# DataZooDE/anofox-forecast

Measured on AMD Instinct MI355X. Metric: series/sec fit+forecast, AutoETS h=28 on M5-shape batches, higher is better.
Workload: dtype f64

## Files before the change

anofox-forecast_amd/csrc/ets_fit_kernel.hpp:

```cpp
#pragma once
#include "ets_device.hpp"
#include "classic_device.hpp"
#include "kernels.hpp"

#ifndef ANOFOX_ROUND_WAVES
#define ANOFOX_ROUND_WAVES 2
#endif
namespace anofox {

#ifndef ANOFOX_PARK_CLASS
#define ANOFOX_PARK_CLASS 0
#endif
#ifndef ANOFOX_PARK_WAVES
#define ANOFOX_PARK_WAVES 4
#endif
#ifndef ANOFOX_DM_WPB
#define ANOFOX_DM_WPB 1
#endif
#ifndef ANOFOX_SETPRIO
#define ANOFOX_SETPRIO 0
#endif
#ifndef ANOFOX_ROUND_WAVES_COMPACT
#define ANOFOX_ROUND_WAVES_COMPACT ANOFOX_ROUND_WAVES
#endif
#ifndef ANOFOX_SEQ_WAVES_COMPACT
#define ANOFOX_SEQ_WAVES_COMPACT 0
#endif
template <class Cfg, class YT = double> struct RoundTraits {
    static constexpr bool DAMPED_MUL = !Cfg::CLASSIC && Cfg::T == C_MUL && Cfg::D;
    static constexpr bool PARK = !Cfg::CLASSIC && (ANOFOX_PARK_CLASS >= 3 || (ANOFOX_PARK_CLASS == 2 && !Cfg::ADDITIVE) || (ANOFOX_PARK_CLASS == 1 && DAMPED_MUL));
    static constexpr int WAVES = PARK ? ANOFOX_PARK_WAVES : (std::is_same_v<YT, double> ? ANOFOX_ROUND_WAVES : ANOFOX_ROUND_WAVES_COMPACT);
    static constexpr int WPB = DAMPED_MUL ? ANOFOX_DM_WPB : 1;
};

template <class Cfg, int MS, class YT = double, bool CLASSIC = Cfg::CLASSIC> struct RoundModelOf { using type = EtsModel<Cfg, MS, 1, YT>; };
template <class Cfg, int MS, class YT> struct RoundModelOf<Cfg, MS, YT, true> { using type = ClassicRoundModel<Cfg::KIND, MS>; };

template <class Cfg, int MS, int SPEC, bool K4 = false, class YT = double>
__device__ __forceinline__ void ets_round_body(const FitArgs &a, const int vblock, const int vgrid, const int wave, double *const lds_all)
{
    constexpr int D = Cfg::DIM;
    constexpr bool PARK = RoundTraits<Cfg>::PARK;
    if constexpr (ANOFOX_SETPRIO >= 1 && RoundTraits<Cfg>::DAMPED_MUL) __builtin_amdgcn_s_setprio(3);
    else if constexpr (ANOFOX_SETPRIO >= 2 && !Cfg::CLASSIC && !Cfg::ADDITIVE) __builtin_amdgcn_s_setprio(ANOFOX_SETPRIO == 2 ? 1 : 2);
    if (a.wave_prio == 3) __builtin_amdgcn_s_setprio(3);
    else if (a.wave_prio == 2) __builtin_amdgcn_s_setprio(2);
    else if (a.wave_prio == 1) __builtin_amdgcn_s_setprio(1);
    if constexpr (Cfg::T == C_MUL && Cfg::D) dm_pow_tab_init();
    const int lane = threadIdx.x & (NM_BLOCK - 1);
    const int lds_per_wave = (PARK ? 0 : nm_lds_doubles<D>()) + ((MS == -1 || MS == -3) ? a.m * NM_BLOCK : 0);
    double *const lds = lds_all + (size_t)wave * (size_t)lds_per_wave;
    double *const nmst = PARK ? a.nm_scratch + (size_t)vblock * (size_t)nm_lds_doubles<D>() : lds;
    double *const lds_ring = PARK ? lds : lds + nm_lds_doubles<D>();
    const unsigned long long trace_t0 = a.wave_trace ? __builtin_amdgcn_s_memrealtime() : 0ull;
    const int n_act = a.n_active ? *a.n_active : a.n_series;
    int mode = SPEC;
    if constexpr (SPEC == 3) mode = n_act > a.spec_below ? 0 : ((a.spec2_below > 0 && n_act <= a.spec2_below && n_act <= vgrid) ? 2 : 1);
    else if (a.spec_below >= 0) {
        const int owner = n_act > a.spec_below ? 0 : (n_act > a.spec2_below ? 1 : 2);
        if (owner != SPEC) return;
    }
    const int LPP = mode == 0 ? 1 : (mode == 1 ? NM_K : NM_BLOCK);
    const int PPB = NM_BLOCK / LPP;
    if (vblock * PPB >= n_act) return;
    const int p = vblock * PPB + lane / LPP;
    const bool valid = p < n_act;
    const int s = valid ? (a.series_of ? a.series_of[p] : p) : 0;
    const int len = valid ? a.len[s] : 0;

    const int m = a.m_col ? (MS <= -3 ? a.m_col[s] : __builtin_amdgcn_readfirstlane(a.m_col[s])) : a.m;
    const int n_param = a.n_param - ((Cfg::S != C_NONE && a.m_col) ? a.m - m : 0);
    bool active = valid;
    if (!a.first_round && a.series_of == nullptr && valid && a.st.done[s]) active = false;
    if (a.first_round) {
        int st = FIT_OK;
        if constexpr (Cfg::CLASSIC) {
            const int min_len = Cfg::KIND == CK_HW ? 2 * m : (Cfg::KIND == CK_SEASONAL_ES ? m : a.min_len);
            if (len <= 0 || (a.mask != nullptr && valid && a.mask[s] != a.want)) st = FIT_SKIPPED;
            else if (len < min_len) st = FIT_SHORT;
        } else {
            const uint32_t fl = valid ? a.flags[s] : 0u;
            if (len <= 0) st = FIT_SKIPPED;
            else if (Cfg::S != C_NONE && len < 2 * m) st = FIT_SHORT;
            else if (len < n_param + 2) st = FIT_SHORT;
            else if (a.need_positive && !(fl & SF_POSITIVE)) st = FIT_NONPOSITIVE;
            else if (a.skip_constant && (fl & SF_CONSTANT)) st = FIT_SKIPPED;
        }
        active = valid && st == FIT_OK;
        if (valid) {
            a.status[s] = st;
            if (!active) { a.st.done[s] = 1; a.st.passes[s] = 0; a.st.evals[s] = 0; a.st.iters[s] = 0; }
        }
    }

    SeriesView v;
// ... 14 lines not shown
    mdl.in.b0 = (active && !Cfg::CLASSIC && Cfg::T != C_NONE) ? a.b0[s] : 0.0;
    mdl.in.fig = a.fig ? a.fig + s : nullptr;
    mdl.in.fig_ld = a.fig_ld;
    mdl.in.m = m;
    mdl.ring = (MS == -2 || MS == -4) ? a.ring_scratch + (size_t)vblock * (size_t)a.m * NM_BLOCK : lds_ring;

    NmRun r;
    if (a.first_round) nm_init_simplex(mdl, nmst, r, active);
    else {
#pragma unroll
        for (int k = 0; k <= D; k++) {
#pragma unroll
            for (int i = 0; i < D; i++) nmst[(k * D + i) * NM_BLOCK + lane] = active ? a.st.sim[(size_t)(k * D + i) * a.ld + s] : 0.0;
            nmst[((D + 1) * D + k) * NM_BLOCK + lane] = active ? a.st.fs[(size_t)k * a.ld + s] : 0.0;
        }
        r.phase = active ? a.st.phase[s] : NM_ITER;
        r.evals = active ? a.st.evals[s] : 0;
        r.iters = active ? a.st.iters[s] : 0;
        r.passes = active ? a.st.passes[s] : 0;
        r.done = !active;
    }
    const int passes_in = r.passes;

    const int budget = mode == 2 ? (1 << 30) : ((SPEC == 3 && mode == 0 && !K4) ? a.budget_seq : a.budget);
#define ANOFOX_ADVANCE_LANE()                                                                          \
    do {                                                                                               \
        if constexpr (K4) {                                                                            \
            EtsModel<Cfg, MS, NM_K, YT> mdl4;                                                          \
            mdl4.v = mdl.v; mdl4.in = mdl.in; mdl4.ring = mdl.ring;                                    \
            nm_advance_spec(mdl4, nmst, r, budget);                                                    \
        } else nm_advance_seq(mdl, nmst, r, budget);                                                   \
    } while (0)
    if constexpr (SPEC == 3) {
        if (mode == 2) nm_advance_spec2(mdl, nmst, r, budget);
        else if (mode == 1) nm_advance_spec(mdl, nmst, r, budget);
        else ANOFOX_ADVANCE_LANE();
    } else if constexpr (SPEC == 2) nm_advance_spec2(mdl, nmst, r, budget);
    else if constexpr (SPEC == 1) nm_advance_spec(mdl, nmst, r, budget);
    else ANOFOX_ADVANCE_LANE();
#undef ANOFOX_ADVANCE_LANE
    nm_fence();

    if (a.wave_trace && lane == 0) {
        const unsigned long long slot = atomicAdd(a.wave_trace, 1ull);
        if (slot < a.wave_trace[1]) {
            unsigned long long *rec = a.wave_trace + 4 + 4 * slot;
            rec[0] = a.wave_trace_tag | ((unsigned long long)mode << 8) | (unsigned long long)(K4 ? 4 : 0);
            rec[1] = trace_t0;
            rec[2] = __builtin_amdgcn_s_memrealtime();
            rec[3] = (unsigned long long)__builtin_amdgcn_s_getreg(0xF804) | ((unsigned long long)__builtin_amdgcn_s_getreg(0xF814) << 32);
        }
    }
    if (a.lane_stats) {
        const int mine = r.passes - passes_in;
        int sum = mine;
#pragma unroll
        for (int o = 32; o >= 1; o >>= 1) sum += __shfl_xor(sum, o);
        const int most = wave_max_i32(mine);
        if (lane == 0 && most > 0) {
            atomicAdd(a.lane_stats, (unsigned long long)most);
            atomicAdd(a.lane_stats + 1, (unsigned long long)sum);
        }
    }
    if (active && (lane % LPP) == 0) {
#pragma unroll
        for (int k = 0; k <= D; k++) {
#pragma unroll
// ... 91 lines not shown
        }
        return;
    }

    if (want_sd && valid && len > 0) a.sd_out[s] = active ? sqrt(var / (double)len) : 0.0;
    if (valid && len > 0) {
        double aicc = __builtin_huge_val();
        if (active) {
            const double lik = f[0];
            if (!(fabs(lik) <= 1.7976931348623157e308)) { st = FIT_NONFINITE; a.status[s] = st; }
            else {
                const double dk = (double)n_param, dn = (double)len;
                const double aic = lik + 2.0 * dk;
                aicc = aic + 2.0 * dk * (dk + 1.0) / (dn - dk - 1.0);
            }
        }
        a.aicc[s] = aicc;
        a.evals[s] = active ? a.st.evals[s] : 0;
        a.iters[s] = active ? a.st.iters[s] : 0;
        a.passes[s] = active ? a.st.passes[s] + 1 : 0;
    }
}

template <class Cfg, int MS, int SPEC, bool K4 = false, class YT = double>
void ets_round_launch(const FitArgs &a, hipStream_t stream)
{
    static_assert(!K4 || ((SPEC == 0 || SPEC == 3) && MS >= 0 && !Cfg::CLASSIC), "K4: the one-lane-per-problem driver of an ETS spec without a run-time ring");
    constexpr int PPB = SPEC == 0 ? NM_BLOCK : (SPEC == 1 ? NM_BLOCK / NM_K : 1);
    int grid;
    if (SPEC == 3) {
        const int n = a.n_series;
        const int g_seq = (n + NM_BLOCK - 1) / NM_BLOCK;
        const int g_spec = (std::min(n, std::max(a.spec_below, 0)) + NM_BLOCK / NM_K - 1) / (NM_BLOCK / NM_K);
        const int g_spec2 = std::min(n, std::max(a.spec2_below, 0));
        grid = std::max(g_seq, std::max(g_spec, g_spec2));
    } else {
        const int n_max = (SPEC == 2 && a.spec_below >= 0 && a.spec2_below < a.n_series) ? a.spec2_below : a.n_series;
        grid = (n_max + PPB - 1) / PPB;
    }
    if (grid <= 0) return;
    constexpr int WPB = RoundTraits<Cfg>::WPB;
    const int blocks = (grid + WPB - 1) / WPB;
    if (RoundTraits<Cfg>::PARK && (a.nm_scratch == nullptr || (size_t)blocks * WPB * (size_t)nm_lds_doubles<Cfg::DIM>() > a.nm_scratch_doubles))
        throw std::runtime_error("ets_round_launch: the simplex scratch does not cover the launch");
    if ((MS == -2 || MS == -4) && (a.ring_scratch == nullptr || (size_t)blocks * WPB * (size_t)a.m * NM_BLOCK > a.ring_scratch_doubles))
        throw std::runtime_error("ets_round_launch: the seasonal-ring scratch does not cover the launch");
    size_t lds_bytes = RoundTraits<Cfg>::PARK ? 0 : sizeof(double) * (size_t)nm_lds_doubles<Cfg::DIM>();
    if (MS == -1 || MS == -3) lds_bytes += sizeof(double) * (size_t)a.m * NM_BLOCK;
    lds_bytes *= WPB;
    if (lds_bytes > 48 * 1024)
        anofox_check_attr(hipFuncSetAttribute((const void *)ets_round_kernel<Cfg, MS, SPEC, K4, YT>, hipFuncAttributeMaxDynamicSharedMemorySize, (int)lds_bytes));
    hipLaunchKernelGGL((ets_round_kernel<Cfg, MS, SPEC, K4, YT>), dim3(blocks), dim3(NM_BLOCK * WPB), lds_bytes, stream, a);
}

template <class Cfg, int MS, class YT = double>
void ets_final_launch(const FitArgs &a, hipStream_t stream)
{
    const int grid = (a.n_series + NM_BLOCK - 1) / NM_BLOCK;
    if (MS == -2 && (a.ring_scratch == nullptr || (size_t)grid * (size_t)a.m * NM_BLOCK > a.ring_scratch_doubles))
        throw std::runtime_error("ets_final_launch: the seasonal-ring scratch does not cover the launch");
    size_t lds_bytes = (MS == -1) ? sizeof(double) * (size_t)a.m * NM_BLOCK : 0;
    hipLaunchKernelGGL((ets_final_kernel<Cfg, MS, YT>), dim3(grid), dim3(NM_BLOCK), lds_bytes, stream, a);
}

}
```

anofox-forecast_amd/csrc/host_api.hip:

```cpp
#include <hip/hip_runtime.h>

#include <algorithm>
#include <cctype>
#include <atomic>
#include <memory>
#include <unordered_map>
#include <chrono>
#include <cmath>
#include <condition_variable>
#include <mutex>
#include <cstdio>
#include <cstdlib>
#include <cstring>
#include <limits>
#include <map>
#include <stdexcept>
#include <string>
#include <system_error>
#include <thread>
#include <vector>

#include "classic_device.hpp"
#include "host_semantics.hpp"
#include "kernels.hpp"
// ... 539 lines not shown
    a.yhat = b->d_yhat; a.status = b->d_detail; a.passes = b->d_passes_total;
    a.model_code = code; a.model_code_out = write_code ? b->d_model_code : nullptr;
    a.ring_scratch = nullptr;
    a.m_col = (kind == CK_HW || kind == CK_SEASONAL_ES) ? b->d_m_col : nullptr;
    const bool optimise = kind == CK_HOLT || kind == CK_HW || optimized != 0;
    if (optimise) {
        const size_t n = b->n, ld = b->ld;
        if (!b->classic_st.sim) {
            b->classic_st.sim = dalloc<double>(12 * ld); b->classic_st.fs = dalloc<double>(4 * ld);
            b->classic_st.phase = dalloc<int32_t>(ld); b->classic_st.evals = dalloc<int32_t>(ld); b->classic_st.iters = dalloc<int32_t>(ld);
            b->classic_st.passes = dalloc<int32_t>(ld); b->classic_st.done = dalloc<int32_t>(ld);
            b->d_classic_status = dalloc<int32_t>(ld);
            b->classic_map[0] = dalloc<int32_t>(ld); b->classic_map[1] = dalloc<int32_t>(ld); b->classic_cnt = dalloc<int32_t>(3);
        }
        double *ybuf = (b->n_slots_cap > 0 && b->use_gather) ? b->lanes[0].ybuf : nullptr;
        size_t ybuf_cols = ybuf ? b->lanes[0].ybuf_cols : ld;
        if (!ybuf) {
            const double per_col = (double)std::max<size_t>(b->t_max, 1) * 8.0;
            const size_t cols = (size_t)std::min((double)ld, 32.0 * 1073741824.0 / per_col) / 64 * 64;
            if (cols >= 1024 || cols >= ld) {
                if (!b->d_classic_ybuf) { b->d_classic_ybuf = dalloc<double>(std::max<size_t>(b->t_max, 1) * cols); b->classic_ybuf_cols = cols; }
                ybuf = b->d_classic_ybuf;
                ybuf_cols = b->classic_ybuf_cols;
            }
        }
        const bool seasonal = kind == CK_HW || kind == CK_SEASONAL_ES;
        FitArgs f{};
        f.y = b->d_y; f.ld = ld; f.len = d_len; f.n_series = (int)n; f.t_rows = (int)std::max<size_t>(b->t_max, 1);
        f.m = seasonal ? std::max(m, 1) : 1; f.h = b->h;
        f.flags = b->d_flags; f.fig = nullptr; f.fig_ld = ld;
        f.status = b->d_classic_status; f.st = b->classic_st;
        f.mask = mask; f.want = want; f.min_len = min_len;
        f.m_col = a.m_col;
        const bool merged = f.m_col != nullptr;
        FitLaunchers fns = classic_fit_launcher(kind, (merged && f.m == 7) ? 8 : f.m);
        if (!fns.round_seq || !fns.round_spec || !fns.round_spec2 || !fns.round_auto) throw HipFail{"no round kernel for this model"};
        if (f.m > ETS_LDS_PERIOD) {
            const size_t wg = merged ? n : std::max<size_t>((n + 15) / 16, std::min<size_t>(n, 1024));
            f.ring_scratch = ensure_ring(b, wg * (size_t)f.m * 64u);
            f.ring_scratch_doubles = wg * (size_t)f.m * 64u;
        }
        static const int BUDGET[] = {24, 24, 24, 24, 48, 48, 96, 192, 1024};
        const bool tiny = n <= TINY_BATCH_PROBLEMS;
        const int n_rounds = tiny ? 1 : (merged ? (n > 4096 ? 4 : 3) : (int)(sizeof BUDGET / sizeof BUDGET[0]));
        for (int r = 0; r < n_rounds; r++) {
            f.first_round = (r == 0);
            f.spec_below = -1; f.spec2_below = -1;
            f.gathered = 0;
            f.y_round = b->d_y; f.ld_round = ld; f.series_of = nullptr; f.n_active = nullptr;
            if (tiny) {
                f.budget = 1 << 30; f.budget_seq = f.budget;
                fns.round_spec2(f, st);
            } else if (merged) {
                f.budget = r == 0 ? 64 : (r == 1 ? 128 : 256); f.budget_seq = f.budget;
                (r < n_rounds - 1 ? fns.round_spec : fns.round_spec2)(f, st);
            } else if (r == 0) {
                const bool seq0 = n >= 4u * 65536u;
                f.budget = seq0 ? (BUDGET[0] * 7) / 4 : BUDGET[0];
                (seq0 ? fns.round_seq : fns.round_spec)(f, st);
            } else {
                int32_t **map = b->classic_map, *cnt = b->classic_cnt;
                const int32_t *prev_map = (r == 1) ? nullptr : map[(r - 1) & 1];
                const int32_t *prev_cnt = (r == 1) ? nullptr : cnt + ((r - 1) % 3);
                if (r == 1) HIPCHECK(hipMemsetAsync(cnt, 0, 3 * sizeof(int32_t), st));
                launch_compact(prev_map, prev_cnt, (int)n, b->classic_st.done, map[r & 1], cnt + (r % 3), st, cnt + ((r + 1) % 3));
                f.series_of = map[r & 1]; f.n_active = cnt + (r % 3);
// ... 196 lines not shown
    std::stable_sort(order.begin(), order.end(), [&](size_t x, size_t y) { return work(specs[x]) > work(specs[y]); });
    std::vector<int> stream_of(order.size());
    for (size_t oi = 0; oi < order.size(); oi++) stream_of[oi] = (int)(oi % (size_t)n_lanes);
    std::vector<FitArgs> args(order.size());
    std::vector<FitLaunchers> fns(order.size());
    for (size_t oi = 0; oi < order.size(); oi++) {
        const size_t k = order[oi];
        const int id = specs[k];
        const int q = (int)(oi % (size_t)n_lanes);
        auto &lane = b->lanes[q];
        const int se = spec_season(id), ti = spec_trend_idx(id);
        const int tt = ti == 0 ? 0 : (ti <= 2 ? 1 : 2);
        FitArgs &a = args[oi];
        a = FitArgs{};
        a.y = (const double *)ybase; a.ld = ld; a.len = d_len; a.n_series = (int)n; a.t_rows = (int)std::max<size_t>(b->t_max, 1);
        a.m = se != 0 ? m : 1; a.h = b->h;
        a.l0 = b->d_l0 + (size_t)(se * 3 + tt) * ld;
        a.b0 = b->d_b0 + (size_t)(se * 3 + tt) * ld;
        a.fig = se == 1 ? b->d_fig_add : (se == 2 ? b->d_fig_mul : nullptr);
        a.fig_ld = ld;
        a.flags = b->d_flags;
        a.need_positive = spec_has_mult(id) ? 1 : 0;
        a.skip_constant = skip_constant ? 1 : 0;
        a.n_param = spec_n_param(id, a.m);
        a.aicc = b->d_aicc + k * ld;
        a.yhat = b->d_yhat_slots + k * n * (size_t)b->h;
        a.status = b->d_status_slots + k * ld;
        a.evals = b->d_evals_slots + k * ld;
        a.iters = b->d_iters_slots + k * ld;
        a.passes = b->d_passes_slots + k * ld;
        a.st = lane.st;
        a.ring_scratch = nullptr;
        a.m_col = b->d_m_col;
        if (b->sd_in_final && order.size() == 1) { a.mean = b->d_mean; a.sd_out = b->d_sd; }
        a.lane_stats = b->d_lane_stats ? b->d_lane_stats + 2 * k : nullptr;
        a.wave_trace = b->d_wave_trace;
        fns[oi] = ets_fit_launcher(id, (merged && se != 0) ? (a.m > lds_limit ? ETS_PERLANE_HBM : ETS_PERLANE_LDS) : a.m, yt);
        if (!fns[oi].round_seq || !fns[oi].round_spec || !fns[oi].round_auto || !fns[oi].final) throw HipFail{"no kernel for ETS spec id " + std::to_string(id)};
    }
    {
        size_t n_long = 0;
        for (size_t oi = 0; oi < order.size(); oi++) if (args[oi].m > lds_limit) n_long++;
        if (n_long) {
            const bool tiny_batch = (uint64_t)n * order.size() <= (uint64_t)TINY_BATCH_PROBLEMS;
            const size_t wg = std::max<size_t>((n + 15) / 16, std::min<size_t>(n, tiny_batch ? n : (size_t)std::max(b->spec2_below, b->spec2_below_md)));
            const size_t per_spec = wg * (size_t)m * 64u;
            if ((double)n_long * (double)per_spec * 8.0 > 64.0 * 1073741824.0)
                throw HipFail{"seasonal period " + std::to_string(m) + " on " + std::to_string(n) + " series needs more than 64 GiB of ring scratch: shard the batch"};
            double *base = ensure_ring(b, n_long * per_spec);
            size_t k = 0;
            for (size_t oi = 0; oi < order.size(); oi++) if (args[oi].m > lds_limit) { args[oi].ring_scratch = base + (k++) * per_spec; args[oi].ring_scratch_doubles = per_spec; }
        }
    }
    {
        const bool tiny_batch = (uint64_t)n * order.size() <= (uint64_t)TINY_BATCH_PROBLEMS;
        const size_t wg = std::max<size_t>((n + 15) / 16, std::min<size_t>(n, tiny_batch ? n : (size_t)std::max(b->spec2_below, b->spec2_below_md)));
        for (size_t oi = 0; oi < order.size(); oi++) {
            if (!fns[oi].nm_scratch_per_wg) continue;
            auto &lane = b->lanes[oi % (size_t)n_lanes];
            const size_t need = (wg + 8) * fns[oi].nm_scratch_per_wg;
            if (lane.nm_scratch_doubles < need) {
                if (lane.nm_scratch) b->retired.push_back(lane.nm_scratch);
                lane.nm_scratch = nullptr; lane.nm_scratch_doubles = 0;
                lane.nm_scratch = dalloc<double>(need);
                lane.nm_scratch_doubles = need;
            }
            args[oi].nm_scratch = lane.nm_scratch; args[oi].nm_scratch_doubles = lane.nm_scratch_doubles;
        }
    }
    std::vector<char> dead(order.size(), 0);
    if (b->none_pos && !b->fixed_params)
        for (size_t oi = 0; oi < order.size(); oi++)
            if (args[oi].need_positive) dead[oi] = 1;
    std::vector<char> k4(order.size(), 0);
    {
        bool all_additive = true;
        for (size_t oi = 0; oi < order.size(); oi++)
            if (!dead[oi] && spec_has_mult(specs[order[oi]]) && !(b->live_all > 0 && b->live_pos >= 0 && 2 * (int64_t)b->live_pos < (int64_t)b->live_all))
                all_additive = false;
        int64_t additive_live = 0;
        for (size_t oi = 0; oi < order.size(); oi++)
            if (!dead[oi] && !spec_has_mult(specs[order[oi]])) additive_live += b->live_all >= 0 ? (int64_t)b->live_all : (int64_t)n;
        int64_t all_live = 0;
        for (size_t oi = 0; oi < order.size(); oi++)
            if (!dead[oi]) all_live += (spec_has_mult(specs[order[oi]]) && b->live_pos >= 0) ? (int64_t)b->live_pos : (b->live_all >= 0 ? (int64_t)b->live_all : (int64_t)n);
        const bool on = b->tun.k4 > 0 || (b->tun.k4 < 0 && yt == YT_F64 && ((all_additive && additive_live >= 131072) || all_live >= 524288));
        for (size_t oi = 0; oi < order.size(); oi++)
            k4[oi] = on && !dead[oi] && !b->fixed_params && !spec_has_mult(specs[order[oi]]) && fns[oi].round_k4 && fns[oi].round_auto_k4;
    }
// ... 92 lines not shown
            if (b->tun.group_split == 2) add_split(of_class[GROUP_GENERAL], GROUP_GENERAL);
            else add(of_class[GROUP_GENERAL], GROUP_GENERAL);
            add(of_class[GROUP_ADDITIVE], GROUP_ADDITIVE);
            grouped = !groups.empty();
        }
        if (grouped) {
            for (size_t g = 0; g < groups.size(); g++) {
                const bool dm = spec_trend_idx(specs[order[groups[g][0]]]) == 4;
                group_stream.push_back(dm ? (int)g : N_AUX_STREAMS - 1 - (int)g);
                for (size_t oi : groups[g]) { group_of[oi] = (int)g; stream_of[oi] = group_stream[g]; slot_of[oi] = n_slots++; }
            }
            for (size_t oi = 0; oi < order.size(); oi++) if (dead[oi]) stream_of[oi] = group_stream[0];
        }
    }
    bool emit = true;
    std::vector<int> slot_blocks, slot_k4;
    GroupCompactArgs gc{};
    GroupGatherArgs gg{};
    int gg_cols = 0;
    auto run_round = [&](const size_t oi, const int kind, const FitArgs &a, hipStream_t sq, const int r) {
        if (!grouped) {
            const FitLaunchFn f = kind == RK_SEQ ? fns[oi].round_seq : kind == RK_SPEC ? fns[oi].round_spec : kind == RK_SPEC2 ? fns[oi].round_spec2 :
                                  kind == RK_AUTO ? fns[oi].round_auto : kind == RK_K4 ? fns[oi].round_k4 : fns[oi].round_auto_k4;
            f(a, sq);
            return;
        }
        if (emit) return;
        FitArgs t = a;
        if (kind == RK_SEQ || kind == RK_K4) { t.spec_below = -1; t.spec2_below = -1; t.budget_seq = t.budget; }
        else if (kind == RK_SPEC) { t.spec_below = 0x7fffffff; t.spec2_below = -1; }
        else if (kind == RK_SPEC2) throw HipFail{"launch_fit_slots: the one-wave-per-problem round of a tiny batch has no group form"};
        const int g_seq = (int)((n + NM_BLOCK - 1) / NM_BLOCK);
        const int g_spec = (int)((std::min<int64_t>((int64_t)n, std::max(t.spec_below, 0)) + NM_BLOCK / NM_K - 1) / (NM_BLOCK / NM_K));
        const int g_spec2 = (int)std::min<int64_t>((int64_t)n, std::max(t.spec2_below, 0));
        const int blocks = std::max(g_seq, std::max(g_spec, g_spec2));
        if (t.ring_scratch != nullptr && (size_t)blocks * (size_t)t.m * NM_BLOCK > t.ring_scratch_doubles)
            throw HipFail{"launch_fit_slots: the seasonal-ring scratch does not cover a group slot"};
        const size_t cell = (size_t)r * n_slots + slot_of[oi];
        b->h_group_tab[cell] = t;
        slot_blocks[cell] = blocks;
        slot_k4[cell] = (kind == RK_K4 || kind == RK_AUTO_K4) ? 1 : 0;
    };
    auto enqueue_round = [&](const int r, const size_t oi) {
            if (dead[oi]) return;
            const int q = (int)(oi % (size_t)n_lanes);
            auto &lane = b->lanes[q];
            hipStream_t sq = spec_stream(stream_of[oi]);
            FitArgs &a = args[oi];
            const bool spec_mode = r >= b->seq_rounds;
            a.first_round = (r == 0);
            a.wave_trace_tag = ((unsigned long long)specs[order[oi]] << 32) | ((unsigned long long)r << 16);
            a.wave_prio = (int)oi < b->tun.prio_top ? std::max(1, 3 - (int)oi) : 0;
            a.spec_below = -1; a.spec2_below = -1;
            a.gathered = 0;
            if (tiny) {
                a.y_round = b->d_y; a.ld_round = ld; a.series_of = nullptr; a.n_active = nullptr;
                a.budget = 1 << 30; a.budget_seq = a.budget;
                run_round(oi, RK_SPEC2, a, sq, r);
                b->fit_launches++;
                return;
            }
            if (r == 0 && b->use_pos && a.need_positive) {
                if (emit)
                    hipLaunchKernelGGL(retire_nonpositive_kernel, dim3((unsigned)((n + 255) / 256)), dim3(256), 0, sq, (int)n, d_len, b->d_notpos,
                                       a.status, lane.st.done, lane.st.passes, lane.st.evals, lane.st.iters);
                a.series_of = b->d_pos_map; a.n_active = b->d_pos_cnt;
                if (b->d_ypos) { a.y_round = b->d_ypos; a.ld_round = ld; a.gathered = 1; a.gather_cap = (int)ld; }
// ... 4513 lines not shown
```

anofox-forecast_amd/csrc/host_resources.hpp:

```cpp
#pragma once

constexpr int N_AUX_STREAMS = 32;

struct HipFail { std::string msg; bool oom = false; };
void report_hip_failure(AnofoxError *out_error, const HipFail &f)
{
    if (f.oom) anofox::set_error(out_error, ALLOCATION_ERROR, "Allocation error: " + f.msg);
    else anofox::set_error(out_error, INTERNAL_ERROR, "Internal error: " + f.msg);
}
#define HIPCHECK(expr)                                                                             \
    do {                                                                                           \
        hipError_t _e = (expr);                                                                    \
        if (_e != hipSuccess) throw HipFail{std::string(#expr) + ": " + hipGetErrorString(_e), _e == hipErrorOutOfMemory};    \
    } while (0)

#define LAUNCHCHECK(what)                                                                          \
    do {                                                                                           \
        hipError_t _e = hipGetLastError();                                                         \
        if (_e != hipSuccess) throw HipFail{std::string("kernel launch failed (") + (what) + "): " + hipGetErrorString(_e), false};    \
    } while (0)

constexpr int32_t STATUS_NOT_COMPUTED = -1;

struct Tunables {
    std::vector<int> budgets{24, 24, 24, 24, 24, 24, 48, 48, 96, 96, 192, 1024};
    int seq_rounds = -1;
    int gather_cols = 0;
    int gather = -1;
    int spec_below = 8192;
    int spec_below_md = 8192;
    int spec2_below = 1024;
    int spec2_below_md = 2048;
    int k4 = -1;
    int k4_top = 1, k4_top_below = 20480;
    std::string wave_trace;
    int compact = -1;
    int fill_policy = 1;
    int fill_target = 150;
    int fill_late_div = 2;
    int fill_s2_div = 16;
    int top_boost_n = 0, top_boost_pct = 200;
    int prio_top = 0;
    int group_launch = 1;
    int group_split = 1;
    int dm_head_rounds = 0;
    bool merge_periods = true;
    int part_threads = 16;
    int pack_threads = 0;
    bool timing = false;
    int arima_trace = 0;
    double arima_lookahead = 6.0;
    int arima_lookahead_depth = 2;
    double arima_spec_factor = 4.0;
    double arima_shared_chunk_rounds = 1.0;
    int arima_prep_lanes = 64;
    int arima_queue_sort = 1;
    int arima_refit_budget = 100;
    static std::map<std::string, std::string> tune_map()
    {
        std::map<std::string, std::string> kv;
        const char *e = std::getenv("ANOFOX_HIP_TUNE");
        if (!e) return kv;
        std::string all(e);
        for (size_t pos = 0; pos < all.size();) {
            size_t end = all.find(';', pos);
// ... 9 lines not shown
            pos = end + 1;
        }
        return kv;
    }
    static Tunables from_env()
    {
        Tunables t;
        const std::map<std::string, std::string> kv = tune_map();
        auto geti = [&](const char *k, int &v) { auto it = kv.find(k); if (it != kv.end()) v = std::atoi(it->second.c_str()); };
        auto getd = [&](const char *k, double &v) { auto it = kv.find(k); if (it != kv.end()) v = std::atof(it->second.c_str()); };
        if (kv.count("budgets")) {
            std::vector<int> v;
            for (const char *q = kv.at("budgets").c_str(); *q;) {
                char *end = nullptr;
                long x = std::strtol(q, &end, 10);
                if (end == q) break;
                if (x > 0) v.push_back((int)x);
                q = (*end == ',') ? end + 1 : end;
            }
            if (!v.empty()) t.budgets = v;
        }
        if (kv.count("wave_trace")) t.wave_trace = kv.at("wave_trace");
        geti("compact", t.compact); geti("prio_top", t.prio_top); geti("top_boost_n", t.top_boost_n); geti("top_boost_pct", t.top_boost_pct);
        geti("fill_policy", t.fill_policy); geti("fill_target", t.fill_target); geti("fill_late_div", t.fill_late_div); geti("fill_s2_div", t.fill_s2_div);
        geti("seq_rounds", t.seq_rounds);
        geti("gather", t.gather);
        if (kv.count("spec_below")) t.spec_below = t.spec_below_md = std::atoi(kv.at("spec_below").c_str());
        geti("spec_below_md", t.spec_below_md);
        geti("gather_cols", t.gather_cols);
        geti("group_launch", t.group_launch); geti("group_split", t.group_split);
        geti("k4", t.k4); geti("dm_head_rounds", t.dm_head_rounds); geti("k4_top", t.k4_top); geti("k4_top_below", t.k4_top_below);
        if (kv.count("spec2_below")) t.spec2_below = t.spec2_below_md = std::atoi(kv.at("spec2_below").c_str());
        geti("spec2_below_md", t.spec2_below_md);
        if (kv.count("merge_periods")) t.merge_periods = std::atoi(kv.at("merge_periods").c_str()) != 0;
        geti("part_threads", t.part_threads);
        if (kv.count("arima_trace")) t.arima_trace = std::atoi(kv.at("arima_trace").c_str());
        getd("arima_lookahead", t.arima_lookahead);
        geti("arima_lookahead_depth", t.arima_lookahead_depth);
        getd("arima_spec_factor", t.arima_spec_factor);
        geti("arima_queue_sort", t.arima_queue_sort);
        geti("arima_prep_lanes", t.arima_prep_lanes);
        getd("arima_shared_chunk_rounds", t.arima_shared_chunk_rounds);
        geti("arima_refit_budget", t.arima_refit_budget);
        if (const char *e = std::getenv("ANOFOX_HIP_PACK_THREADS")) t.pack_threads = std::max(1, std::atoi(e));
        t.timing = std::getenv("ANOFOX_HIP_TIMING") != nullptr;
        return t;
    }
};
struct ProcessTunables {
    double cache_gb = -1.0, pinned_cache_gb = 2.0;
    double coalesce_us = 1000.0;
    int prio_streams = -1;
    std::string devices;
    static const ProcessTunables &get()
    {
        static const ProcessTunables t = [] {
            ProcessTunables p;
            if (const char *e = std::getenv("ANOFOX_HIP_CACHE_GB")) p.cache_gb = std::atof(e);
            if (const char *e = std::getenv("ANOFOX_HIP_PINNED_CACHE_GB")) p.pinned_cache_gb = std::atof(e);
            { const auto kv = Tunables::tune_map(); auto it = kv.find("prio_streams"); if (it != kv.end()) p.prio_streams = std::atoi(it->second.c_str()); }
            if (const char *e = std::getenv("ANOFOX_HIP_COALESCE_US")) p.coalesce_us = std::atof(e);
            if (const char *e = std::getenv("ANOFOX_HIP_DEVICES")) p.devices = e;
            return p;
        }();
        return t;
    }
// ... 423 lines not shown
```

anofox-forecast_amd/csrc/kernels.hpp:

```cpp
#pragma once
#include <hip/hip_runtime.h>
#include <stddef.h>
#include <stdint.h>
#include <atomic>

#include <stdexcept>
#include <string>

namespace anofox {

inline void anofox_check_attr(hipError_t e)
{
    if (e != hipSuccess) throw std::runtime_error(std::string("launch preparation failed: ") + hipGetErrorString(e));
}

enum : uint32_t { SF_POSITIVE = 1u, SF_CONSTANT = 2u, SF_HAS_NAN = 4u };

enum : int32_t { FIT_OK = 0, FIT_SHORT = 1, FIT_NONPOSITIVE = 2, FIT_NONFINITE = 3, FIT_PERIOD = 4, FIT_SKIPPED = 5 };

struct PrepArgs {
    const double *y; size_t ld; const int32_t *len; int n_series;
    int m;
    const int32_t *m_col;
    double *mean, *sd;
    uint32_t *flags;
    double *fig_add, *fig_mul;
    double *l0, *b0;
    double *scratch;
    int pre_fig;
    int t_rows;
    int skip_sd;
    int skip_types;
};

size_t season_scratch_doubles(int n_series, int t_rows, int m_max);
void launch_season_figures(const PrepArgs &a, hipStream_t stream);

struct NmStateBuf {
    double *sim;
    double *fs;
    int32_t *phase, *evals, *iters, *passes, *done;
};

struct FitArgs {
    const double *y; size_t ld; const int32_t *len; int n_series;
    int t_rows;
    const double *y_round; size_t ld_round;
    const int32_t *series_of;
    const int32_t *n_active;
    int budget, first_round;
    const int32_t *m_col;
    int spec_below;
    const uint32_t *mask;
    uint32_t want;
    int min_len;
    int budget_seq;
    int spec2_below;
    int gathered;
    int gather_cap;
    NmStateBuf st;
    double *ring_scratch;
    size_t ring_scratch_doubles;
    double *nm_scratch;
    size_t nm_scratch_doubles;
    int m, h;
    const double *l0, *b0;
    const double *fig; size_t fig_ld;
    const uint32_t *flags;
    int need_positive;
    int skip_constant;
    int n_param;
    double *aicc;
    double *yhat;
    int32_t *status;
    int32_t *evals, *iters, *passes;
    const int32_t *insp_sel;
    int32_t insp_code;
    double *insp_fitted;
    double *insp_states;
    double *insp_info;
    unsigned long long *lane_stats;
    const double *mean;
    double *sd_out;
    int wave_prio;
    unsigned long long *wave_trace;
    unsigned long long wave_trace_tag;
};

struct SelectArgs {
    int n_series, h, n_slots;
    size_t ld;
    const int32_t *len;
    const double *aicc;
    const double *yhat_slots;
    const int32_t *slot_spec;
    const int32_t *status_slots;
    const int32_t *passes_slots;
    const int32_t *evals_slots;
    double *yhat;
    int32_t *model_code;
    int32_t *status;
    uint32_t *fallback_mask;
    int32_t *passes_total;
    int32_t *evals_total;
};

struct ClassicArgs {
    const double *y; size_t ld; const int32_t *len; int n_series;
    int m, h;
    int optimized;
    double fixed_alpha;
    const uint32_t *mask;
    uint32_t want;
    int min_len;
    double *yhat;
    int32_t *status;
    int32_t *passes;
    int32_t model_code;
    int32_t *model_code_out;
    double *ring_scratch;
    const int32_t *m_col;
// ... 312 lines not shown
```

anofox-forecast_amd/csrc/nm.hpp:

```cpp
#pragma once
#include <hip/hip_runtime.h>

namespace anofox {

constexpr int NM_K = 4;
constexpr int NM_BLOCK = 64;

__device__ __forceinline__ double nm_clip(double v, double lo, double hi)
{
    if (v < lo) v = lo;
    if (v > hi) v = hi;
    return v;
}

enum { NM_INIT0 = 0, NM_INIT1 = 1, NM_ITER = 2, NM_SHRINK = 3, NM_SEQ_INIT = 4, NM_SEQ_E = 5, NM_SEQ_OC = 6, NM_SEQ_IC = 7, NM_SEQ_SHRINK = 8 };

struct NmRun { int phase; int evals; int iters; int passes; bool done; };
struct NmStats { int iters; int evals; int passes; };

template <int D> constexpr int nm_lds_doubles() { return ((D + 1) * D + (D + 1)) * NM_BLOCK; }

template <int D> struct NmSimplex { double x[D + 1][D]; double f[D + 1]; };

template <int D> __device__ __forceinline__ void nm_load(const double *st, int lane, NmSimplex<D> &S)
// ... 250 lines not shown
        }
        s = pos == 0 ? v : s + v;
    }
    const double xb = s / (double)D;
    const double xw = j == D ? xp : S.x[D - 1][i];
    const double a = which == 0 ? 2.0 : (which == 1 ? 3.0 : (which == 2 ? 1.5 : 0.5));
    const double b = which == 0 ? 1.0 : (which == 1 ? 2.0 : 0.5);
    const double t = which == 3 ? a * xb + b * xw : a * xb - b * xw;
    return nm_clip(t, lo, hi);
}

template <int D> __device__ __forceinline__ bool nm_decide(const NmSimplex<D> &S, const double (&fc)[NM_K], int &evals, int &which, double &fnew)
{
    const double fxr = fc[0];
    evals += 1;
    which = 0;
    fnew = fxr;
    if (fxr < S.f[0]) {
        evals += 1;
        if (fc[1] < fxr) { which = 1; fnew = fc[1]; }
        return true;
    }
    if (fxr < S.f[D - 1]) return true;
    if (fxr < S.f[D]) {
        evals += 1;
        if (fc[2] <= fxr) { which = 2; fnew = fc[2]; return true; }
        return false;
    }
    evals += 1;
    if (fc[3] < S.f[D]) { which = 3; fnew = fc[3]; return true; }
    return false;
}

template <class Model>
__device__ void nm_advance_spec2(Model &mdl, double *st, NmRun &r, int budget)
{
    constexpr int D = Model::DIM;
    constexpr int NH = 3 * D + 3;
    const int lane = threadIdx.x & (NM_BLOCK - 1);
    double lo[D], hi[D], x0[D];
    mdl.bounds(lo, hi, x0);
    const int maxiter = 200 * D, maxfun = 200 * D;
    int phase = r.phase, evals = r.evals, iters = r.iters, passes = r.passes;
    bool done = r.done, parked = false;
    const int hh = lane >= NM_K ? (lane - NM_K) >> 2 : 0, w2 = (lane - NM_K) & 3;
    int hp = 0, hj = 0;
    nm_hypothesis<D>(hh < NH ? hh : 0, hp, hj);
    double x[D];

    for (int pass = 0;; pass++) {
        if (!done && !parked) {
            NmSimplex<D> S;
            nm_load<D>(st, lane, S);
            const int sub = lane < NM_K ? lane : NM_K - 1;
            if (phase == NM_INIT0) {
#pragma unroll
                for (int i = 0; i < D; i++) x[i] = nm_store_x<D>(st, lane, sub <= D ? sub : D, i);
            } else if (phase == NM_INIT1) {
#pragma unroll
                for (int i = 0; i < D; i++) x[i] = S.x[D][i];
            } else if (phase == NM_ITER) {
                if (!(evals < maxfun && iters < maxiter)) done = true;
                else if (nm_converged<D>(S)) done = true;
                if (!done) {
                    if (lane < NM_K) {
#pragma unroll
                        for (int i = 0; i < D; i++) x[i] = nm_trial<D>(S, lane, i, lo[i], hi[i]);
                    } else {
#pragma unroll
                        for (int i = 0; i < D; i++) x[i] = nm_trial2<D>(S, hp, hj, w2, i, lo[i], hi[i]);
                    }
                }
            } else {
#pragma unroll
                for (int i = 0; i < D; i++) x[i] = nm_store_x<D>(st, lane, sub + 1 <= D ? sub + 1 : D, i);
            }
        }
        if (!done && pass >= budget && (phase == NM_ITER || phase == NM_INIT0)) parked = true;
        if (done || parked) break;

        const double f = mdl.eval1(x);
        passes += 1;
        nm_fence();
        double fc[NM_K];
#pragma unroll
        for (int k = 0; k < NM_K; k++) fc[k] = __shfl(f, k);

        NmSimplex<D> S;
        nm_load<D>(st, lane, S);
        if (phase == NM_INIT0) {
#pragma unroll
            for (int k = 0; k < NM_K; k++)
                if (k <= D) S.f[k] = fc[k];
            evals += (D + 1 < NM_K ? D + 1 : NM_K);
            phase = (D + 1 > NM_K) ? NM_INIT1 : NM_ITER;
            if (phase == NM_ITER) nm_sort_all<D>(S);
        } else if (phase == NM_INIT1) {
            S.f[D] = fc[0];
            evals += 1;
            phase = NM_ITER;
            nm_sort_all<D>(S);
        } else if (phase == NM_ITER) {
            int which = 0;
            double fnew = 0.0;
            if (!nm_decide<D>(S, fc, evals, which, fnew)) {
                nm_shrink_vertices<D>(S, lo, hi);
                phase = NM_SHRINK;
            } else {
                int j = D;
#pragma unroll
                for (int k = D; k >= 1; k--)
                    if (j == k && fnew < S.f[k - 1]) j = k - 1;
                const int hstar = which == 1 ? 0 : (which == 0 ? 1 + j : (which == 2 ? D + 1 + j : 2 * D + 2 + j));
                double fc2[NM_K];
#pragma unroll
                for (int k = 0; k < NM_K; k++) fc2[k] = __shfl(f, NM_K + 4 * hstar + k);
                nm_accept<D>(S, which, fnew, lo, hi);
                iters += 1;
                if (!(evals < maxfun && iters < maxiter) || nm_converged<D>(S)) done = true;
                else if (NM_K + 4 * NH <= NM_BLOCK) {
                    if (!nm_decide<D>(S, fc2, evals, which, fnew)) {
                        nm_shrink_vertices<D>(S, lo, hi);
                        phase = NM_SHRINK;
                    } else {
                        nm_accept<D>(S, which, fnew, lo, hi);
                        iters += 1;
                    }
                }
            }
        } else {
#pragma unroll
            for (int k = 0; k < NM_K; k++)
                if (k + 1 <= D) S.f[k + 1] = fc[k];
            evals += D;
            iters += 1;
            phase = NM_ITER;
            nm_sort_all<D>(S);
        }
        nm_store<D>(st, lane, S);
    }
    r.phase = phase; r.evals = evals; r.iters = iters; r.passes = passes; r.done = done;
}

template <class Model>
__device__ void nm_advance_seq(Model &mdl, double *st, NmRun &r, int budget)
{
    constexpr int D = Model::DIM;
    const int lane = threadIdx.x & (NM_BLOCK - 1);
    double lo[D], hi[D], x0[D];
    mdl.bounds(lo, hi, x0);
    const int maxiter = 200 * D, maxfun = 200 * D;
    int phase = r.phase, evals = r.evals, iters = r.iters, passes = r.passes;
    bool done = r.done, parked = false;
    int vi = 0;
    double fxr = 0.0;
    double x[D];

    for (int pass = 0;; pass++) {
        if (!done && !parked) {
            if (phase == NM_INIT0) { phase = NM_SEQ_INIT; vi = 0; }
            if (phase == NM_SEQ_INIT || phase == NM_SEQ_SHRINK) {
                const int k = phase == NM_SEQ_INIT ? vi : 1 + vi;
#pragma unroll
                for (int i = 0; i < D; i++) x[i] = nm_store_x<D>(st, lane, k, i);
            } else {
                NmSimplex<D> S;
                nm_load<D>(st, lane, S);
                if (phase == NM_ITER) {
                    if (!(evals < maxfun && iters < maxiter)) done = true;
                    else if (nm_converged<D>(S)) done = true;
                }
                const int which = phase == NM_ITER ? 0 : (phase == NM_SEQ_E ? 1 : (phase == NM_SEQ_OC ? 2 : 3));
// ... 83 lines not shown
```

Before: 79560.

## Pack two Nelder-Mead problems per wave in spec2 mode with ranked hypotheses

The speculative two-step Nelder-Mead driver can now run two problems per 64-lane wave, 32 lanes each. Because a half wave cannot hold every second-step hypothesis, hypotheses are ordered by a ranked table so the likeliest ones get lanes, and the second step is skipped when the chosen hypothesis is uncovered. Host grid sizing and scratch allocation use a new helper that halves the workgroup count. This packs more problems per wave in the tail phase, at the cost of fewer speculative second steps and a wave-level loop exit that keeps finished halves idle until both are done.

```diff
diff --git a/anofox-forecast_amd/csrc/ets_fit_kernel.hpp b/anofox-forecast_amd/csrc/ets_fit_kernel.hpp
--- a/anofox-forecast_amd/csrc/ets_fit_kernel.hpp
+++ b/anofox-forecast_amd/csrc/ets_fit_kernel.hpp
@@ -55,12 +55,16 @@
     const unsigned long long trace_t0 = a.wave_trace ? __builtin_amdgcn_s_memrealtime() : 0ull;
     const int n_act = a.n_active ? *a.n_active : a.n_series;
     int mode = SPEC;
-    if constexpr (SPEC == 3) mode = n_act > a.spec_below ? 0 : ((a.spec2_below > 0 && n_act <= a.spec2_below && n_act <= vgrid) ? 2 : 1);
-    else if (a.spec_below >= 0) {
+    int lp2 = NM_BLOCK;
+    if constexpr (SPEC == 3) {
+        lp2 = (a.spec2_lanes == NM_BLOCK / 2 && n_act > a.spec2_full_below) ? NM_BLOCK / 2 : NM_BLOCK;
+        const int ppb2 = NM_BLOCK / lp2;
+        mode = n_act > a.spec_below ? 0 : ((a.spec2_below > 0 && n_act <= a.spec2_below && (n_act + ppb2 - 1) / ppb2 <= vgrid) ? 2 : 1);
+    } else if (a.spec_below >= 0) {
         const int owner = n_act > a.spec_below ? 0 : (n_act > a.spec2_below ? 1 : 2);
         if (owner != SPEC) return;
     }
-    const int LPP = mode == 0 ? 1 : (mode == 1 ? NM_K : NM_BLOCK);
+    const int LPP = mode == 0 ? 1 : (mode == 1 ? NM_K : lp2);
     const int PPB = NM_BLOCK / LPP;
     if (vblock * PPB >= n_act) return;
     const int p = vblock * PPB + lane / LPP;
@@ -141,7 +145,7 @@
         } else nm_advance_seq(mdl, nmst, r, budget);                                                   \
     } while (0)
     if constexpr (SPEC == 3) {
-        if (mode == 2) nm_advance_spec2(mdl, nmst, r, budget);
+        if (mode == 2) nm_advance_spec2(mdl, nmst, r, budget, lp2);
         else if (mode == 1) nm_advance_spec(mdl, nmst, r, budget);
         else ANOFOX_ADVANCE_LANE();
     } else if constexpr (SPEC == 2) nm_advance_spec2(mdl, nmst, r, budget);
@@ -299,7 +303,7 @@
         const int n = a.n_series;
         const int g_seq = (n + NM_BLOCK - 1) / NM_BLOCK;
         const int g_spec = (std::min(n, std::max(a.spec_below, 0)) + NM_BLOCK / NM_K - 1) / (NM_BLOCK / NM_K);
-        const int g_spec2 = std::min(n, std::max(a.spec2_below, 0));
+        const int g_spec2 = spec2_workgroups(n, a.spec2_below, a.spec2_lanes, a.spec2_full_below);
         grid = std::max(g_seq, std::max(g_spec, g_spec2));
     } else {
         const int n_max = (SPEC == 2 && a.spec_below >= 0 && a.spec2_below < a.n_series) ? a.spec2_below : a.n_series;
diff --git a/anofox-forecast_amd/csrc/host_api.hip b/anofox-forecast_amd/csrc/host_api.hip
--- a/anofox-forecast_amd/csrc/host_api.hip
+++ b/anofox-forecast_amd/csrc/host_api.hip
@@ -595,6 +595,7 @@
         f.status = b->d_classic_status; f.st = b->classic_st;
         f.mask = mask; f.want = want; f.min_len = min_len;
         f.m_col = a.m_col;
+        f.spec2_lanes = b->tun.spec2_lanes == 32 ? 32 : 64; f.spec2_full_below = b->tun.spec2_full_below;
         const bool merged = f.m_col != nullptr;
         FitLaunchers fns = classic_fit_launcher(kind, (merged && f.m == 7) ? 8 : f.m);
         if (!fns.round_seq || !fns.round_spec || !fns.round_spec2 || !fns.round_auto) throw HipFail{"no round kernel for this model"};
@@ -857,6 +858,7 @@
         a.st = lane.st;
         a.ring_scratch = nullptr;
         a.m_col = b->d_m_col;
+        a.spec2_lanes = b->tun.spec2_lanes == 32 ? 32 : 64; a.spec2_full_below = b->tun.spec2_full_below;
         if (b->sd_in_final && order.size() == 1) { a.mean = b->d_mean; a.sd_out = b->d_sd; }
         a.lane_stats = b->d_lane_stats ? b->d_lane_stats + 2 * k : nullptr;
         a.wave_trace = b->d_wave_trace;
@@ -868,7 +870,7 @@
         for (size_t oi = 0; oi < order.size(); oi++) if (args[oi].m > lds_limit) n_long++;
         if (n_long) {
             const bool tiny_batch = (uint64_t)n * order.size() <= (uint64_t)TINY_BATCH_PROBLEMS;
-            const size_t wg = std::max<size_t>((n + 15) / 16, std::min<size_t>(n, tiny_batch ? n : (size_t)std::max(b->spec2_below, b->spec2_below_md)));
+            const size_t wg = std::max<size_t>((n + 15) / 16, tiny_batch ? n : (size_t)spec2_workgroups((long long)n, std::max(b->spec2_below, b->spec2_below_md), b->tun.spec2_lanes, b->tun.spec2_full_below));
             const size_t per_spec = wg * (size_t)m * 64u;
             if ((double)n_long * (double)per_spec * 8.0 > 64.0 * 1073741824.0)
                 throw HipFail{"seasonal period " + std::to_string(m) + " on " + std::to_string(n) + " series needs more than 64 GiB of ring scratch: shard the batch"};
@@ -879,7 +881,7 @@
     }
     {
         const bool tiny_batch = (uint64_t)n * order.size() <= (uint64_t)TINY_BATCH_PROBLEMS;
-        const size_t wg = std::max<size_t>((n + 15) / 16, std::min<size_t>(n, tiny_batch ? n : (size_t)std::max(b->spec2_below, b->spec2_below_md)));
+        const size_t wg = std::max<size_t>((n + 15) / 16, tiny_batch ? n : (size_t)spec2_workgroups((long long)n, std::max(b->spec2_below, b->spec2_below_md), b->tun.spec2_lanes, b->tun.spec2_full_below));
         for (size_t oi = 0; oi < order.size(); oi++) {
             if (!fns[oi].nm_scratch_per_wg) continue;
             auto &lane = b->lanes[oi % (size_t)n_lanes];
@@ -1038,7 +1040,7 @@
         else if (kind == RK_SPEC2) throw HipFail{"launch_fit_slots: the one-wave-per-problem round of a tiny batch has no group form"};
         const int g_seq = (int)((n + NM_BLOCK - 1) / NM_BLOCK);
         const int g_spec = (int)((std::min<int64_t>((int64_t)n, std::max(t.spec_below, 0)) + NM_BLOCK / NM_K - 1) / (NM_BLOCK / NM_K));
-        const int g_spec2 = (int)std::min<int64_t>((int64_t)n, std::max(t.spec2_below, 0));
+        const int g_spec2 = spec2_workgroups((long long)n, t.spec2_below, t.spec2_lanes, t.spec2_full_below);
         const int blocks = std::max(g_seq, std::max(g_spec, g_spec2));
         if (t.ring_scratch != nullptr && (size_t)blocks * (size_t)t.m * NM_BLOCK > t.ring_scratch_doubles)
             throw HipFail{"launch_fit_slots: the seasonal-ring scratch does not cover a group slot"};
diff --git a/anofox-forecast_amd/csrc/host_resources.hpp b/anofox-forecast_amd/csrc/host_resources.hpp
--- a/anofox-forecast_amd/csrc/host_resources.hpp
+++ b/anofox-forecast_amd/csrc/host_resources.hpp
@@ -31,6 +31,8 @@
     int spec_below_md = 8192;
     int spec2_below = 1024;
     int spec2_below_md = 2048;
+    int spec2_lanes = 32;
+    int spec2_full_below = 0;
     int k4 = -1;
     int k4_top = 1, k4_top_below = 20480;
     std::string wave_trace;
@@ -106,6 +108,7 @@
         geti("k4", t.k4); geti("dm_head_rounds", t.dm_head_rounds); geti("k4_top", t.k4_top); geti("k4_top_below", t.k4_top_below);
         if (kv.count("spec2_below")) t.spec2_below = t.spec2_below_md = std::atoi(kv.at("spec2_below").c_str());
         geti("spec2_below_md", t.spec2_below_md);
+        geti("spec2_lanes", t.spec2_lanes); geti("spec2_full_below", t.spec2_full_below);
         if (kv.count("merge_periods")) t.merge_periods = std::atoi(kv.at("merge_periods").c_str()) != 0;
         geti("part_threads", t.part_threads);
         if (kv.count("arima_trace")) t.arima_trace = std::atoi(kv.at("arima_trace").c_str());
diff --git a/anofox-forecast_amd/csrc/kernels.hpp b/anofox-forecast_amd/csrc/kernels.hpp
--- a/anofox-forecast_amd/csrc/kernels.hpp
+++ b/anofox-forecast_amd/csrc/kernels.hpp
@@ -2,6 +2,7 @@
 #include <hip/hip_runtime.h>
 #include <stddef.h>
 #include <stdint.h>
+#include <algorithm>
 #include <atomic>
 
 #include <stdexcept>
@@ -56,6 +57,8 @@
     int min_len;
     int budget_seq;
     int spec2_below;
+    int spec2_lanes;
+    int spec2_full_below;
     int gathered;
     int gather_cap;
     NmStateBuf st;
@@ -87,6 +90,14 @@
     unsigned long long wave_trace_tag;
 };
 
+inline int spec2_workgroups(long long n, int spec2_below, int spec2_lanes, int spec2_full_below)
+{
+    const long long top = std::min<long long>(n, std::max(spec2_below, 0));
+    if (spec2_lanes != 32) return (int)top;
+    const long long full = std::min<long long>(top, std::max(spec2_full_below, 0));
+    return (int)std::max<long long>(full, (top + 1) / 2);
+}
+
 struct SelectArgs {
     int n_series, h, n_slots;
     size_t ld;
diff --git a/anofox-forecast_amd/csrc/nm.hpp b/anofox-forecast_amd/csrc/nm.hpp
--- a/anofox-forecast_amd/csrc/nm.hpp
+++ b/anofox-forecast_amd/csrc/nm.hpp
@@ -306,27 +306,77 @@
     return false;
 }
 
+template <int D> struct NmRank;
+template <> struct NmRank<1> { static constexpr int order[6] = {5, 4, 0, 1, 2, 3}; };
+template <> struct NmRank<2> { static constexpr int order[9] = {6, 0, 2, 7, 8, 1, 4, 3, 5}; };
+template <> struct NmRank<3> { static constexpr int order[12] = {0, 8, 2, 9, 1, 3, 10, 5, 11, 4, 6, 7}; };
+template <> struct NmRank<4> { static constexpr int order[15] = {0, 2, 10, 11, 1, 3, 4, 12, 13, 6, 7, 5, 8, 14, 9}; };
+
+template <int D> constexpr int nm_rank_slot(int h)
+{
+    for (int q = 0; q < 3 * D + 3; q++)
+        if (NmRank<D>::order[q] == h) return q;
+    return 3 * D + 3;
+}
+template <int D> constexpr bool nm_rank_is_permutation()
+{
+    for (int h = 0; h < 3 * D + 3; h++) {
+        int n = 0;
+        for (int q = 0; q < 3 * D + 3; q++) n += NmRank<D>::order[q] == h ? 1 : 0;
+        if (n != 1) return false;
+    }
+    return true;
+}
+template <int D> constexpr unsigned long long nm_rank_pack()
+{
+    unsigned long long w = 0;
+    for (int q = 0; q < 3 * D + 3; q++) w |= (unsigned long long)NmRank<D>::order[q] << (4 * q);
+    return w;
+}
+template <int D> constexpr unsigned long long nm_rank_inverse_pack()
+{
+    unsigned long long w = 0;
+    for (int h = 0; h < 3 * D + 3; h++) w |= (unsigned long long)nm_rank_slot<D>(h) << (4 * h);
+    return w;
+}
+template <int D> constexpr bool nm_rank_inverse_matches()
+{
+    for (int h = 0; h < 3 * D + 3; h++) {
+        const int q = (int)((nm_rank_inverse_pack<D>() >> (4 * h)) & 15ull);
+        if (q >= 3 * D + 3 || (int)((nm_rank_pack<D>() >> (4 * q)) & 15ull) != h) return false;
+    }
+    return true;
+}
+static_assert(nm_rank_is_permutation<1>() && nm_rank_is_permutation<2>() && nm_rank_is_permutation<3>() && nm_rank_is_permutation<4>(),
+              "every ranked hypothesis list is a permutation of 0 .. 3 D + 2");
+static_assert(nm_rank_inverse_matches<1>() && nm_rank_inverse_matches<2>() && nm_rank_inverse_matches<3>() && nm_rank_inverse_matches<4>(),
+              "the hypothesis -> slot table is the inverse of the ranked list");
+
 template <class Model>
-__device__ void nm_advance_spec2(Model &mdl, double *st, NmRun &r, int budget)
+__device__ void nm_advance_spec2(Model &mdl, double *st, NmRun &r, int budget, const int LP = NM_BLOCK)
 {
     constexpr int D = Model::DIM;
     constexpr int NH = 3 * D + 3;
+    static_assert(NM_K + 4 * NH <= NM_BLOCK, "a whole wave holds every hypothesis");
     const int lane = threadIdx.x & (NM_BLOCK - 1);
+    const int gl = lane & (LP - 1), base = lane - gl;
+    const int n_slots = (LP - NM_K) >> 2;
     double lo[D], hi[D], x0[D];
     mdl.bounds(lo, hi, x0);
     const int maxiter = 200 * D, maxfun = 200 * D;
     int phase = r.phase, evals = r.evals, iters = r.iters, passes = r.passes;
     bool done = r.done, parked = false;
-    const int hh = lane >= NM_K ? (lane - NM_K) >> 2 : 0, w2 = (lane - NM_K) & 3;
+    const int slot = gl >= NM_K ? (gl - NM_K) >> 2 : 0, w2 = (gl - NM_K) & 3;
+    const int hh = slot < NH ? (int)((nm_rank_pack<D>() >> (4 * slot)) & 15ull) : 0;
     int hp = 0, hj = 0;
-    nm_hypothesis<D>(hh < NH ? hh : 0, hp, hj);
+    nm_hypothesis<D>(hh, hp, hj);
     double x[D];
 
     for (int pass = 0;; pass++) {
         if (!done && !parked) {
             NmSimplex<D> S;
             nm_load<D>(st, lane, S);
-            const int sub = lane < NM_K ? lane : NM_K - 1;
+            const int sub = gl < NM_K ? gl : NM_K - 1;
             if (phase == NM_INIT0) {
 #pragma unroll
                 for (int i = 0; i < D; i++) x[i] = nm_store_x<D>(st, lane, sub <= D ? sub : D, i);
@@ -337,9 +387,9 @@
                 if (!(evals < maxfun && iters < maxiter)) done = true;
                 else if (nm_converged<D>(S)) done = true;
                 if (!done) {
-                    if (lane < NM_K) {
-#pragma unroll
-                        for (int i = 0; i < D; i++) x[i] = nm_trial<D>(S, lane, i, lo[i], hi[i]);
+                    if (gl < NM_K) {
+#pragma unroll
+                        for (int i = 0; i < D; i++) x[i] = nm_trial<D>(S, gl, i, lo[i], hi[i]);
                     } else {
 #pragma unroll
                         for (int i = 0; i < D; i++) x[i] = nm_trial2<D>(S, hp, hj, w2, i, lo[i], hi[i]);
@@ -351,67 +401,71 @@
             }
         }
         if (!done && pass >= budget && (phase == NM_ITER || phase == NM_INIT0)) parked = true;
-        if (done || parked) break;
+        if (__all(done || parked)) break;
 
         const double f = mdl.eval1(x);
-        passes += 1;
+        passes += (done || parked) ? 0 : 1;
         nm_fence();
         double fc[NM_K];
 #pragma unroll
-        for (int k = 0; k < NM_K; k++) fc[k] = __shfl(f, k);
-
-        NmSimplex<D> S;
-        nm_load<D>(st, lane, S);
-        if (phase == NM_INIT0) {
-#pragma unroll
-            for (int k = 0; k < NM_K; k++)
-                if (k <= D) S.f[k] = fc[k];
-            evals += (D + 1 < NM_K ? D + 1 : NM_K);
-            phase = (D + 1 > NM_K) ? NM_INIT1 : NM_ITER;
-            if (phase == NM_ITER) nm_sort_all<D>(S);
-        } else if (phase == NM_INIT1) {
-            S.f[D] = fc[0];
-            evals += 1;
-            phase = NM_ITER;
-            nm_sort_all<D>(S);
-        } else if (phase == NM_ITER) {
-            int which = 0;
-            double fnew = 0.0;
-            if (!nm_decide<D>(S, fc, evals, which, fnew)) {
-                nm_shrink_vertices<D>(S, lo, hi);
-                phase = NM_SHRINK;
+        for (int k = 0; k < NM_K; k++) fc[k] = __shfl(f, base + k);
+
+        if (!done && !parked) {
+            NmSimplex<D> S;
+            nm_load<D>(st, lane, S);
+            if (phase == NM_INIT0) {
+#pragma unroll
+                for (int k = 0; k < NM_K; k++)
+                    if (k <= D) S.f[k] = fc[k];
+                evals += (D + 1 < NM_K ? D + 1 : NM_K);
+                phase = (D + 1 > NM_K) ? NM_INIT1 : NM_ITER;
+                if (phase == NM_ITER) nm_sort_all<D>(S);
+            } else if (phase == NM_INIT1) {
+                S.f[D] = fc[0];
+                evals += 1;
+                phase = NM_ITER;
+                nm_sort_all<D>(S);
+            } else if (phase == NM_ITER) {
+                int which = 0;
+                double fnew = 0.0;
+                if (!nm_decide<D>(S, fc, evals, which, fnew)) {
+                    nm_shrink_vertices<D>(S, lo, hi);
+                    phase = NM_SHRINK;
+                } else {
+                    int j = D;
+#pragma unroll
+                    for (int k = D; k >= 1; k--)
+                        if (j == k && fnew < S.f[k - 1]) j = k - 1;
+                    const int hstar = which == 1 ? 0 : (which == 0 ? 1 + j : (which == 2 ? D + 1 + j : 2 * D + 2 + j));
+                    const int sstar = (int)((nm_rank_inverse_pack<D>() >> (4 * hstar)) & 15ull);
+                    const bool covered = sstar < n_slots;
+                    double fc2[NM_K];
+#pragma unroll
+                    for (int k = 0; k < NM_K; k++) fc2[k] = __shfl(f, base + NM_K + 4 * (covered ? sstar : 0) + k);
+                    nm_accept<D>(S, which, fnew, lo, hi);
+                    iters += 1;
+                    if (!(evals < maxfun && iters < maxiter) || nm_converged<D>(S)) done = true;
+                    else if (covered) {
+                        if (!nm_decide<D>(S, fc2, evals, which, fnew)) {
+                            nm_shrink_vertices<D>(S, lo, hi);
+                            phase = NM_SHRINK;
+                        } else {
+                            nm_accept<D>(S, which, fnew, lo, hi);
+                            iters += 1;
+                        }
+                    }
+                }
             } else {
-                int j = D;
-#pragma unroll
-                for (int k = D; k >= 1; k--)
-                    if (j == k && fnew < S.f[k - 1]) j = k - 1;
-                const int hstar = which == 1 ? 0 : (which == 0 ? 1 + j : (which == 2 ? D + 1 + j : 2 * D + 2 + j));
-                double fc2[NM_K];
-#pragma unroll
-                for (int k = 0; k < NM_K; k++) fc2[k] = __shfl(f, NM_K + 4 * hstar + k);
-                nm_accept<D>(S, which, fnew, lo, hi);
+#pragma unroll
+                for (int k = 0; k < NM_K; k++)
+                    if (k + 1 <= D) S.f[k + 1] = fc[k];
+                evals += D;
                 iters += 1;
-                if (!(evals < maxfun && iters < maxiter) || nm_converged<D>(S)) done = true;
-                else if (NM_K + 4 * NH <= NM_BLOCK) {
-                    if (!nm_decide<D>(S, fc2, evals, which, fnew)) {
-                        nm_shrink_vertices<D>(S, lo, hi);
-                        phase = NM_SHRINK;
-                    } else {
-                        nm_accept<D>(S, which, fnew, lo, hi);
-                        iters += 1;
-                    }
-                }
-            }
-        } else {
-#pragma unroll
-            for (int k = 0; k < NM_K; k++)
-                if (k + 1 <= D) S.f[k + 1] = fc[k];
-            evals += D;
-            iters += 1;
-            phase = NM_ITER;
-            nm_sort_all<D>(S);
-        }
-        nm_store<D>(st, lane, S);
+                phase = NM_ITER;
+                nm_sort_all<D>(S);
+            }
+            nm_store<D>(st, lane, S);
+        }
     }
     r.phase = phase; r.evals = evals; r.iters = iters; r.passes = passes; r.done = done;
 }
```

New measurement: 80300 (median of 6 runs). Within noise of the previous version (+0.9%).
